# HilaManor/AudioEditingCode

Measured on AMD Instinct MI355X. Metric: edited-clips/sec (200-step inv+edit, 10 s@16 kHz), higher is better.
Workload: dtype f32

## Files before the change

audioeditingcode_amd/csrc/elementwise.hip:

```cpp
#include "aed_common.h"

static inline int grid_for(size_t n, int per_thread = 1) {
    size_t g = (n + 256 * (size_t)per_thread - 1) / (256 * (size_t)per_thread);
    if (g > 4096) g = 4096;
    if (g < 1) g = 1;
    return (int)g;
}

__global__ __launch_bounds__(256) void copy2d_kernel(const float* __restrict__ src, float* __restrict__ dst, int rows,
                                                      int cols, int lds_, int ldd, int vec, const int* state,
                                                      int idx_off, int idx_mul, long idx_stride, const float* coef,
                                                      int c_mul, int c_off, int c_stride, int c_col) {
    const int st = state ? state[0] : 0;
    if (state) src += (size_t)(idx_off + idx_mul * st) * (size_t)idx_stride;
    const float sc = coef ? coef[(size_t)(st * c_mul + c_off) * c_stride + c_col] : 1.0f;
    if (vec) {
        const int q = cols >> 2;
        const size_t total = (size_t)rows * q;
        for (size_t e = (size_t)blockIdx.x * 256 + threadIdx.x; e < total; e += (size_t)gridDim.x * 256) {
            const int r = (int)(e / q);
            const int c = (int)(e - (size_t)r * q) * 4;
            float4 v = *reinterpret_cast<const float4*>(src + (size_t)r * lds_ + c);
            if (coef) { v.x *= sc; v.y *= sc; v.z *= sc; v.w *= sc; }
            *reinterpret_cast<float4*>(dst + (size_t)r * ldd + c) = v;
        }
    } else {
        const size_t total = (size_t)rows * cols;
        for (size_t e = (size_t)blockIdx.x * 256 + threadIdx.x; e < total; e += (size_t)gridDim.x * 256) {
            const int r = (int)(e / cols);
            const int c = (int)(e - (size_t)r * cols);
            const float v = src[(size_t)r * lds_ + c];
            dst[(size_t)r * ldd + c] = coef ? v * sc : v;
        }
    }
}
int launch_copy2d(const aed_op* op, hipStream_t s) {
    const int32_t* i = op->i;
    AED_REQUIRE(op->p[0] && op->p[1], "copy2d: null pointer");
    const int vec = (i[1] % 4 == 0) && (i[2] % 4 == 0) && (i[3] % 4 == 0) && ((uintptr_t)op->p[0] % 16 == 0) &&
                    ((uintptr_t)op->p[1] % 16 == 0) && (i[6] % 4 == 0);
    hipLaunchKernelGGL(copy2d_kernel, dim3(grid_for((size_t)i[0] * i[1] / (vec ? 4 : 1))), dim3(256), 0, s,
                       (const float*)op->p[0], (float*)op->p[1], i[0], i[1], i[2], i[3], vec, (const int*)op->p[2],
                       i[4], i[5], (long)i[6], (const float*)op->p[3], i[7], i[8], i[9], i[10]);
    AED_CHECK_HIP(hipGetLastError());
    return 0;
}

__global__ void time_embed_kernel(float* out, const long long* tt, const int* state, const float* freqs,
                                  const int* row_tidx, int B, int dim, int flip, int ld, int t_imm, int tgroup,
                                  float shift, float max_period, int float_table) {
    const int half = dim / 2;
    const int s = state ? state[0] : 0;
    for (int e = blockIdx.x * blockDim.x + threadIdx.x; e < B * half; e += gridDim.x * blockDim.x) {
        const int b = e / half, i = e - b * half;
        const int ti = s * tgroup + (row_tidx ? row_tidx[b] : 0);
        const float t = !tt ? (float)t_imm : float_table ? reinterpret_cast<const float*>(tt)[ti] : (float)tt[ti];
        const float fr = freqs ? freqs[i] : expf(-logf(max_period) * (float)i / ((float)half - shift));
        const float arg = t * fr;
        const float sv = sinf(arg), cv = cosf(arg);
        float* o = out + (size_t)b * ld;
        if (flip) { o[i] = cv; o[half + i] = sv; }
        else { o[i] = sv; o[half + i] = cv; }
    }
}
int launch_time_embed(const aed_op* op, hipStream_t s) {
    const int32_t* i = op->i;
    AED_REQUIRE(op->p[0] && i[1] % 2 == 0, "time_embed: bad args");
    hipLaunchKernelGGL(time_embed_kernel, dim3(aed_cdiv(i[0] * i[1] / 2, 256)), dim3(256), 0, s, (float*)op->p[0],
                       (const long long*)op->p[1], (const int*)op->p[2], (const float*)op->p[3], (const int*)op->p[4],
                       i[0], i[1], i[2], i[3], i[4], i[5] > 0 ? i[5] : 1, op->f[0],
                       op->f[1] > 0.f ? op->f[1] : 10000.0f, i[6]);
    AED_CHECK_HIP(hipGetLastError());
    return 0;
}

__global__ __launch_bounds__(256) void softmax_rows_kernel(const float* __restrict__ x, float* __restrict__ y, int cols,
                                                            int ldx, int ldy, float scale) {
    __shared__ float red[4];
    const int row = blockIdx.x, tid = threadIdx.x;
    const float* xr = x + (size_t)row * ldx;
    float* yr = y + (size_t)row * ldy;
    float m = -INFINITY;
    for (int c = tid; c < cols; c += 256) m = fmaxf(m, xr[c] * scale);
    for (int o = 32; o > 0; o >>= 1) m = fmaxf(m, __shfl_xor(m, o, 64));
    if ((tid & 63) == 0) red[tid >> 6] = m;
    __syncthreads();
    m = fmaxf(fmaxf(red[0], red[1]), fmaxf(red[2], red[3]));
    __syncthreads();
    float sum = 0.f;
    for (int c = tid; c < cols; c += 256) {
        const float e = expf(xr[c] * scale - m);
        yr[c] = e;
        sum += e;
    }
    for (int o = 32; o > 0; o >>= 1) sum += __shfl_xor(sum, o, 64);
    if ((tid & 63) == 0) red[tid >> 6] = sum;
    __syncthreads();
    sum = (red[0] + red[1]) + (red[2] + red[3]);
    const float inv = 1.0f / sum;
    for (int c = tid; c < cols; c += 256) yr[c] *= inv;
}
int launch_softmax_rows(const aed_op* op, hipStream_t s) {
    const int32_t* i = op->i;
    AED_REQUIRE(op->p[0] && op->p[1], "softmax_rows: null pointer");
    hipLaunchKernelGGL(softmax_rows_kernel, dim3(i[0]), dim3(256), 0, s, (const float*)op->p[0], (float*)op->p[1], i[1],
                       i[2], i[3], op->f[0]);
    AED_CHECK_HIP(hipGetLastError());
    return 0;
}

__global__ __launch_bounds__(256) void transpose_kernel(const float* __restrict__ src, float* __restrict__ dst, int R,
                                                         int C, int lds_, int ldd, long bs_src, long bs_dst) {
    __shared__ float tile[32][33];
    const float* s = src + (size_t)blockIdx.z * bs_src;
    float* d = dst + (size_t)blockIdx.z * bs_dst;
    const int tx = threadIdx.x & 31, ty = threadIdx.x >> 5;
    const int r0 = blockIdx.y * 32, c0 = blockIdx.x * 32;
    for (int j = ty; j < 32; j += 8) {
        const int r = r0 + j, c = c0 + tx;
        tile[j][tx] = (r < R && c < C) ? s[(size_t)r * lds_ + c] : 0.f;
    }
    __syncthreads();
    for (int j = ty; j < 32; j += 8) {
        const int c = c0 + j, r = r0 + tx;
// ... 762 lines not shown
```

audioeditingcode_amd/editing.py:

```python
import math

import torch

from . import _lib as L
from .scheduler import coefficient_table, step_coefficients
from . import tape as tape_mod
from .tape import Tape
from .unet import PackedUNetWeights, UNetEngine

PAD_BIAS = -1.0e30
MASK_BIAS = -10000.0


class Conditioning:

    def __init__(self, ehs0=None, ehs1=None, mask0=None, mask1=None, class_labels=None):
        self.ehs0, self.ehs1, self.mask0, self.mask1, self.class_labels = ehs0, ehs1, mask0, mask1, class_labels

    @property
    def rows(self):
        for t in (self.ehs0, self.ehs1, self.class_labels):
            if t is not None:
                return t.shape[0]
        return 0

    def repeat(self, n):
        f = lambda t: None if t is None else t.repeat_interleave(n, 0) if t.shape[0] == 1 else t
        return Conditioning(f(self.ehs0), f(self.ehs1), f(self.mask0), f(self.mask1), f(self.class_labels))

    def select(self, rows):
        f = lambda t: None if t is None else t[list(rows)]
        return Conditioning(f(self.ehs0), f(self.ehs1), f(self.mask0), f(self.mask1), f(self.class_labels))


def _pad_ctx(parts, L, attr_e, attr_m):
    es, bs = [], []
    dev0 = getattr(parts[0], attr_e).device
    for c in parts:
        e = getattr(c, attr_e).float().to(dev0)
        m = getattr(c, attr_m)
        r, l, d = e.shape
        ep = torch.zeros(r, L, d, dtype=torch.float32, device=e.device)
        ep[:, :l] = e
        b = torch.full((r, L), PAD_BIAS, dtype=torch.float32, device=e.device)
        b[:, :l] = 0.0 if m is None else (1 - m.float().to(e.device)) * MASK_BIAS
        es.append(ep)
        bs.append(b)
    return torch.cat(es, 0), torch.cat(bs, 0)


def variant_plan(tstarts, n_zs, max_variants=None):
    ts = [int(t) for t in tstarts]
    if not ts:
        raise ValueError("edit_variants: the list of variants is empty")
    if max_variants is not None and len(ts) > max_variants:
        raise ValueError(f"edit_variants: {len(ts)} variants in one call, at most {max_variants} "
                         f"(variants.inversion_reverse_variants splits longer lists)")
    for t in ts:
        if not 1 <= t <= n_zs:
            raise ValueError(f"edit_variants: tstart {t} outside [1, {n_zs}] (the number of noise maps zs holds)")
    order = sorted(range(len(ts)), key=lambda v: -ts[v])
    segs, i = [], 0
    while i < len(order):
        j = i
        while j < len(order) and ts[order[j]] == ts[order[i]]:
            j += 1
        segs.append(dict(tstart=ts[order[i]], a=j, join=(i, j)))
        i = j
    for k, sg in enumerate(segs):
        nxt = segs[k + 1]["tstart"] if k + 1 < len(segs) else 0
        sg["start"], sg["steps"] = segs[0]["tstart"] - sg["tstart"], sg["tstart"] - nxt
    return order, segs


def variant_positions(order):
    pos = [0] * len(order)
    for i, v in enumerate(order):
        pos[v] = i
    return pos


def variant_noise(eta_rows):
    if isinstance(eta_rows, float):
        return eta_rows > 0
    if any(e == 0 for e in eta_rows) and any(e != 0 for e in eta_rows):
        raise ValueError("edit_variants: a per-step eta list that is zero at some steps and non-zero at others is not "
                         "supported by the device loop; use inversion_reverse_process per variant")
    return any(e > 0 for e in eta_rows)


# ... 267 lines not shown
                        with lock:
                            g = Tape.graph_capture(body)
                    if plan is not None:
                        plan["graph"] = g
                ev0.record(stream)
                chooser = getattr(self, "lane_chooser", None)
                if chooser is None:
                    for _ in range(steps):
                        Tape.graph_replay(g)
                else:
                    stream = self._replay_in_chunks(g, steps, stream, chooser)
                ev1.record(stream)
                self._last_events = (ev0, ev1)
                if plan is None:
                    stream.synchronize()
                    L.check(L.lib().aed_graph_destroy(g), "aed_graph_destroy")
            else:
                ev0.record(stream)
                for _ in range(steps):
                    body()
                ev1.record(stream)
                self._last_events = (ev0, ev1)
        cur.wait_stream(stream)

    LANE_CHUNK = 5

    def _replay_in_chunks(self, g, steps, stream, chooser):
        pending, cur_s, done = [], stream, 0
        while done < steps:
            if len(pending) >= 2:
                pending.pop(0).synchronize()
            s = chooser() or stream
            if s is not cur_s:
                hand = torch.cuda.Event()
                hand.record(cur_s)
                s.wait_event(hand)
                cur_s = s
            n = min(self.LANE_CHUNK, steps - done)
            with torch.cuda.stream(cur_s):
                for _ in range(n):
                    Tape.graph_replay(g)
            ev = torch.cuda.Event()
            ev.record(cur_s)
            pending.append(ev)
            done += n
        return cur_s

    def last_loop_ms(self):
        ev0, ev1 = self._last_events
        ev1.synchronize()
        return ev0.elapsed_time(ev1)


class EditEngine(LoopPlumbing):
    def __init__(self, unet_cfg, weights, scheduler, device, H, W, kind):
        self.cfg, self.sched, self.device = unet_cfg, scheduler, torch.device(device)
        self.H, self.W, self.C = H, W, unet_cfg["in_channels"]
        self.kind = kind
        self.weights = weights if isinstance(weights, PackedUNetWeights) else PackedUNetWeights(weights, device)
        self.stream = torch.cuda.Stream(device=self.device) if self.device.type == "cuda" else None
        self._unets = {}
        self.state = torch.zeros(4, dtype=torch.int32, device=self.device)
        self.ts_dev = torch.zeros(scheduler.config.num_train_timesteps, dtype=torch.int64, device=self.device)
        self._ts_host = None
        self._plans = {}
        self.max_plans = 8

    def _upload_timesteps(self, ts, n):
        ts = ts.detach().to("cpu", torch.int64).reshape(-1)[:n].clone()
        if self._ts_host is not None and self._ts_host.numel() >= n and torch.equal(self._ts_host[:n], ts):
            return
        self.ts_dev[:n] = ts.to(self.device)
        self._ts_host = ts

    arith = "bf16x6"
    ARITH_MIN_BATCH = 2

    def _arith_for(self, B):
        return self.arith if B >= self.ARITH_MIN_BATCH else "f32"

    SHARE_CFG_ROWS = True
    SHARE_IN_EDIT_LOOP = True

    def unet(self, B, L0=0, L1=0, share=1):
        arith = self._arith_for(B)
        share = int(share) if (self.SHARE_CFG_ROWS and share > 1 and self.kind != "audioldm") else 1
        key = (B, L0, L1) if arith == "f32" else (B, L0, L1, arith)
        if share > 1:
            key = key + (f"share{share}",)
        if key not in self._unets:
            with tape_mod.arith_mode(arith):
                self._unets[key] = UNetEngine(self.cfg, self.weights, self.device, B, self.H, self.W, ctx_len0=L0,
                                              ctx_len1=L1, use_ehs=self.kind != "audioldm",
                                              timesteps_dev=self.ts_dev, state_dev=self.state, share=share)
        return self._unets[key]

    def _set_cond(self, eng, groups, repeat=1):
        tile = (lambda t: t) if repeat == 1 else (lambda t: t.repeat(repeat, *([1] * (t.dim() - 1))))
        if self.kind == "audioldm":
            d0 = groups[0].class_labels.device
            eng.set_conditioning(class_labels=tile(torch.cat([g.class_labels.float().to(d0) for g in groups], 0)))
        elif self.kind == "audioldm2":
            d0 = groups[0].ehs0.device
            e0 = torch.cat([g.ehs0.float().to(d0) for g in groups], 0)
            e1, b1 = _pad_ctx(groups, eng.L1, "ehs1", "mask1")
            eng.set_conditioning(ehs0=tile(e0), ehs1=tile(e1), bias1=tile(b1))
        else:
            e0, b0 = _pad_ctx(groups, eng.L0, "ehs0", "mask0")
            eng.set_conditioning(ehs0=tile(e0), bias0=tile(b0))

    def _coef_table(self, s, ts, eta, kind):
        key = (kind, tuple(int(t) for t in ts), tuple(eta) if isinstance(eta, (list, tuple)) else float(eta),
               int(s.config.num_train_timesteps), int(s.num_inference_steps), str(s.config.prediction_type),
               float(s.alphas_cumprod[0]), float(s.alphas_cumprod[-1]), float(s.final_alpha_cumprod))
        cache = self.__dict__.setdefault("_coef_cache", {})
        tab = cache.pop(key, None)
        if tab is None:
            tab = coefficient_table(s, ts, eta=eta, kind=kind)
            while len(cache) >= 8:
                cache.pop(next(iter(cache)))
        cache[key] = tab
        return tab

    @staticmethod
    def _round_len(n):
        for p2 in (8, 16, 32):
            if n <= p2:
                return p2
        return n

    def _ctx_lens(self, groups):
        if self.kind == "audioldm":
            return 0, 0
        if self.kind == "audioldm2":
            return groups[0].ehs0.shape[1], self._round_len(max(g.ehs1.shape[1] for g in groups))
        return self._round_len(max(g.ehs0.shape[1] for g in groups)), 0

    @torch.inference_mode()
    def to_nhwc(self, x, out=None):
        lead = x.shape[:-3]
        C, H, W = x.shape[-3:]
        src = x.to(self.device, torch.float32).contiguous()
        dst = out if out is not None else torch.empty(*lead, H, W, C, device=self.device, dtype=torch.float32)
        tp = Tape(self.device)
        tp.transpose(src, dst, Bt=max(1, math.prod(lead)), R=C, C=H * W)
        tp.run()
        return dst

    @torch.inference_mode()
    def to_nchw(self, x):
        lead = x.shape[:-3]
        H, W, C = x.shape[-3:]
        src = x.contiguous()
        dst = torch.empty(*lead, C, H, W, device=self.device, dtype=torch.float32)
        tp = Tape(self.device)
        tp.transpose(src, dst, Bt=max(1, math.prod(lead)), R=H * W, C=C)
        tp.run()
        return dst

    @torch.inference_mode()
    def sample_xts(self, x0, noise=None, generator=None):
        s = self.sched
        T = s.num_inference_steps
        x0 = x0.to(self.device, torch.float32).contiguous()
        if noise is None:
            noise = torch.stack([torch.randn(x0.shape, generator=generator, dtype=torch.float32) for _ in range(T)])
        noise = noise.to(self.device, torch.float32).contiguous()
        ts = s.timesteps.cpu()
        abar = s.alphas_cumprod
        t_rows = torch.stack([ts[T - (r + 1)] for r in range(T)])
        sa = (abar[t_rows] ** 0.5).to(self.device)
        sb = ((1 - abar) ** 0.5)[t_rows].to(self.device)
        xts = torch.empty((T + 1, *x0.shape), device=self.device, dtype=torch.float32)
        xts[0] = x0
        L.check(L.lib().aed_sample_xts_from_x0(x0.data_ptr(), noise.data_ptr(), sa.data_ptr(), sb.data_ptr(),
                                                xts[1:].data_ptr(), T, x0.numel(), L.current_stream_ptr()),
                "aed_sample_xts_from_x0")
        return xts

    @staticmethod
    def _etas_in_loop_order(eta, n_rows):
        if not isinstance(eta, (list, tuple)) and not (torch.is_tensor(eta) and eta.dim() > 0):
            return float(eta)
        etas = [float(e) for e in eta]
        if len(etas) < n_rows:
            raise ValueError(f"{len(etas)} eta values for {n_rows} steps")
        return [etas[n_rows - 1 - k] for k in range(n_rows)]

    @torch.inference_mode()
    def invert(self, x0, cond_src, cond_uncond, cfg_src, eta=1.0, numerical_fix=True, noise=None, generator=None,
               xts=None, cfg_tensor=None, mode="sequential", group=8, use_graph=True):
        s = self.sched
        T = s.num_inference_steps
        n = x0.shape[0]
        numel = n * self.C * self.H * self.W
        if xts is None:
            xts = self.sample_xts(x0, noise, generator)
        P = 0 if cond_src is None else cond_src.rows // n
        groups = [cond_uncond.repeat(n)] + ([cond_src] if P else [])
        v_pred = int(s.config.prediction_type == "v_prediction")
        G = 1 if mode == "sequential" else max(1, min(group, T))
        while T % G:
            G -= 1
        rows_per_t = n * (1 + P)
        L0, L1 = self._ctx_lens(groups)
        scalar = float(cfg_src[0]) if (cfg_tensor is None and P) else 1.0
        key = ("invert", n, P, T, G, L0, L1, bool(numerical_fix), v_pred, cfg_tensor is not None, scalar,
               self._arith_for(G * rows_per_t))
        plan = self._get_plan(key)
        if plan is None:
            plan = self._plans[key] = dict(
                state=torch.zeros(4, dtype=torch.int32, device=self.device),
                xts=torch.empty((T + 1, n, self.H, self.W, self.C), device=self.device, dtype=torch.float32),
                zs=torch.zeros((T, n, self.H, self.W, self.C), device=self.device, dtype=torch.float32),
                coef=torch.zeros((T, L.COEF_STRIDE), device=self.device, dtype=torch.float32),
                cfgt=(torch.empty((max(P, 1), n, self.H, self.W, self.C), device=self.device, dtype=torch.float32)
                      if cfg_tensor is not None else None))
            eng = plan["eng"] = self.unet(G * rows_per_t, L0, L1, share=(1 + P) if (n == 1 and G >= 2) else 1)
            pre, post = Tape(self.device), Tape(self.device)
            for g in range(G):
                for blk in range(1 + P):
                    dst = eng.x_in[(g * (1 + P) + blk) * n:(g * (1 + P) + blk + 1) * n]
                    pre.copy2d(plan["xts"], dst, rows=1, cols=numel, ld_src=numel, ld_dst=numel, state=plan["state"],
                               idx_off=T - g, idx_mul=-G, idx_stride=numel, name="x_in<-xts")
            for g in range(G):
                base = g * rows_per_t
                eps_u = eng.eps[base:base + n]
                eps_c = eng.eps[base + n:base + rows_per_t] if P else None
                post.step(L.OP_INVERT_STEP, xts=plan["xts"], zs=plan["zs"], eps_u=eps_u, eps_c=eps_c,
                          cfg=plan["cfgt"], coef=plan["coef"], state=plan["state"], out=None, numel=numel, P=max(P, 1),
                          T=T, v_pred=v_pred, flag=int(numerical_fix), cfg_scalar=scalar, s_mul=G, s_off=g)
            post.advance(plan["state"])
            pre.finalize()
            post.finalize()
            plan["pre"], plan["post"] = pre, post
        eng, pre, post = plan["eng"], plan["pre"], plan["post"]
        xts = self.to_nhwc(xts, out=plan["xts"])
        zs = plan["zs"]
        plan["coef"].copy_(self._coef_table(s, s.timesteps.cpu(), self._etas_in_loop_order(eta, T), "ddpm"))
        self._upload_timesteps(s.timesteps, T)
        if cfg_tensor is not None:
            self.to_nhwc(cfg_tensor.reshape(P, n, self.C, self.H, self.W), out=plan["cfgt"])
        self._set_cond(eng, groups, repeat=G)
        self._patch_time(eng, self.ts_dev, G, rows_per_t, state=plan["state"])
        plan["state"].zero_()

        def body():
            pre.run()
            eng.tape.run()
            post.run()
        self._run_graph(body, T // G, use_graph, plan)
        zs[0].zero_()
        return zs, xts

    def _patch_time(self, eng, ts_dev, G, rows_per_t, offset=0, state=None):
        state = self.state if state is None else state
        op = eng.tape.ops[eng.time_op]
        arr = eng.tape.finalize()
        cache = eng.__dict__.setdefault("_row_tidx_cache", {})
        if rows_per_t not in cache:
            cache[rows_per_t] = (torch.arange(eng.B, dtype=torch.int32) // max(1, rows_per_t)).to(self.device)
        eng._row_tidx = cache[rows_per_t]
        for o in (op, arr[eng.time_op]):
            o.p[1] = ts_dev.data_ptr() + 8 * offset
            o.p[2] = state.data_ptr()
            o.p[4] = eng._row_tidx.data_ptr()
            o.i[5] = G

    @torch.inference_mode()
    def edit(self, xts, zs, tstart, cond_tgt, cond_neg, cfg_tar, eta=1.0, cfg_tensor=None, use_graph=True,
             table_kind="ddpm", n_steps=None):
        s = self.sched
        T = s.num_inference_steps
        n = xts.shape[1]
        numel = n * self.C * self.H * self.W
        Z = int(tstart)
        P = cond_tgt.rows // n
        groups = [cond_neg.repeat(n), cond_tgt]
        ts = s.timesteps.cpu()[T - Z:]
        v_pred = int(s.config.prediction_type == "v_prediction")
        scalar = float(cfg_tar[0]) if cfg_tensor is None else 1.0
        L0, L1 = self._ctx_lens(groups)
        eta_rows = self._etas_in_loop_order(eta, Z)
        any_noise = (eta_rows > 0) if isinstance(eta_rows, float) else any(e > 0 for e in eta_rows)
        has_noise = int(any_noise and zs is not None)
        key = ("edit", n, P, T, Z, L0, L1, v_pred, cfg_tensor is not None, scalar, has_noise, table_kind,
               self._arith_for(n * (1 + P)))
        plan = self._get_plan(key)
        if plan is None:
            plan = self._plans[key] = dict(
                state=torch.zeros(4, dtype=torch.int32, device=self.device),
                cur=torch.empty((n, self.H, self.W, self.C), device=self.device, dtype=torch.float32),
                zs=torch.zeros((Z, n, self.H, self.W, self.C), device=self.device, dtype=torch.float32),
                coef=torch.zeros((Z, L.COEF_STRIDE), device=self.device, dtype=torch.float32),
                cfgt=(torch.empty((P, n, self.H, self.W, self.C), device=self.device, dtype=torch.float32)
                      if cfg_tensor is not None else None))
            eng = plan["eng"] = self.unet(n * (1 + P), L0, L1, share=(1 + P) if (n == 1 and self.SHARE_IN_EDIT_LOOP) else 1)
            pre, post = Tape(self.device), Tape(self.device)
            for blk in range(1 + P):
                pre.copy2d(plan["cur"], eng.x_in[blk * n:(blk + 1) * n], rows=1, cols=numel, ld_src=numel,
                           ld_dst=numel, name="x_in<-x_t")
            post.step(L.OP_REVERSE_STEP, xts=plan["cur"], zs=plan["zs"] if has_noise else None, eps_u=eng.eps[:n],
                      eps_c=eng.eps[n:], cfg=plan["cfgt"], coef=plan["coef"], state=plan["state"], out=plan["cur"],
                      numel=numel, P=P, T=Z if has_noise else 0, v_pred=v_pred, flag=has_noise, cfg_scalar=scalar)
            post.advance(plan["state"])
            pre.finalize()
            post.finalize()
            plan["pre"], plan["post"] = pre, post
        eng, pre, post, cur = plan["eng"], plan["pre"], plan["post"], plan["cur"]
        cur.copy_(xts[Z])
        if has_noise:
            plan["zs"].copy_(zs[:Z])
        plan["coef"].copy_(self._coef_table(s, ts, eta_rows, table_kind))
        self._upload_timesteps(s.timesteps, T)
        if cfg_tensor is not None:
            self.to_nhwc(cfg_tensor.reshape(P, n, self.C, self.H, self.W), out=plan["cfgt"])
        self._set_cond(eng, groups)
        self._patch_time(eng, self.ts_dev, 1, n * (1 + P), offset=T - Z, state=plan["state"])
        plan["state"].zero_()

        def body():
            pre.run()
            eng.tape.run()
            post.run()
        self._run_graph(body, Z if n_steps is None else max(0, min(int(n_steps), Z)), use_graph, plan)
        return cur.clone()

    MAX_VARIANTS = 16

    def _variant_loop(self, tag, order, segs, tgt, neg, cfgs, eta, noise_ok, fill_noise, join_rows, use_graph, src=None,
                      n_tables=0, drift=None, n_steps=None, rowsel=None, seg=None):
        s = self.sched
        T = s.num_inference_steps
        K = len(order)
        Z0 = segs[0]["tstart"]
        eta_rows = self._etas_in_loop_order(eta, Z0)
        has_noise = int(variant_noise(eta_rows) and noise_ok)
        numel = self.C * self.H * self.W
        v_pred = int(s.config.prediction_type == "v_prediction")
        P = 1 if seg is None else seg["P"]
        B = 1 + P
        groups_all = [neg[v] for v in order] + ([tgt[v] for v in order] if seg is None else
                                                [tgt[v].select([j]) for j in range(P) for v in order])
        L0, L1 = self._ctx_lens(groups_all)
        tables = () if src is None else (n_tables,)
        R = None if rowsel is None else len(rowsel["coefs"])
        rkey = () if rowsel is None else (n_tables, R)
        if rowsel is not None:
            tables = (max(n_tables, 1),)
        dkey = () if drift is None else (tuple(drift["vecs"].shape[:2]), drift["s_first"], bool(drift["shift_np"]),
                                          drift["fix_mode"], float(drift["fix_alpha"]))
        key = (tag, K, *(tables if rowsel is None else ()), T, tuple(sg["tstart"] for sg in segs),
               tuple(sg["a"] for sg in segs), L0, L1, v_pred, has_noise,
               tuple(self._arith_for(B * sg["a"]) for sg in segs), *dkey, *rkey, *(() if seg is None else (P,)))
        plan = self._get_plan(key)
        if plan is None:
            plan = self._plans[key] = dict(
                state=torch.zeros(4, dtype=torch.int32, device=self.device),
                cur=torch.empty((K, self.H, self.W, self.C), device=self.device, dtype=torch.float32),
                zs=torch.zeros((*tables, Z0, self.H, self.W, self.C), device=self.device, dtype=torch.float32),
                coef=torch.zeros((*(() if R is None else (R,)), Z0, L.COEF_STRIDE), device=self.device, dtype=torch.float32),
                cfg=torch.zeros(K, device=self.device, dtype=torch.float32),
                src=None if src is None else torch.zeros(K, device=self.device, dtype=torch.int32), segs=[])
            if rowsel is not None:
                plan["rowsel"] = torch.zeros((2, K), device=self.device, dtype=torch.int32)
            if drift is not None:
                S, n_ev = drift["vecs"].shape[:2]
                dev_buf = lambda *shape: torch.zeros(shape, device=self.device, dtype=torch.float32)
                plan.update(vecs=dev_buf(S, n_ev, self.H, self.W, self.C), w=dev_buf(S, K, n_ev),
                            mask=dev_buf(self.H, self.W, self.C) if drift["fix_mode"] else None,
                            par=dev_buf(T + 1, self.H, self.W, self.C) if drift["fix_mode"] == 1 else None)
            if seg is not None:
                lat = (self.H, self.W, self.C)
                plan.update(cfg=torch.zeros((K, P, *lat), device=self.device, dtype=torch.float32),
                            mask=torch.zeros((K, P, *lat), device=self.device, dtype=torch.float32),
                            lag=torch.zeros((K, P), device=self.device, dtype=torch.int32),
                            alpha=torch.zeros(K, device=self.device, dtype=torch.float32),
                            traj=torch.zeros((Z0, *lat), device=self.device, dtype=torch.float32))
            for sg in segs:
                a = sg["a"]
                eng = self.unet(B * a, L0, L1, share=1)
                pre, post = Tape(self.device), Tape(self.device)
# ... 397 lines not shown
```

audioeditingcode_amd/unet.py:

```python
import torch

from . import _lib as L
from .tape import Tape
from .weights import ctx_dims_per_block, _per_block


TWO_SOURCE = True
MERGE_FF2_PROJ = True
FOLD_XATTN = True


def geglu_pack_index(dff):
    q = torch.arange(dff // 32)[:, None]
    j = torch.arange(32)[None, :]
    return torch.cat([32 * q + j, dff + 32 * q + j], 1).reshape(-1)


class PackedUNetWeights:

    def __init__(self, sd, device):
        self.device = torch.device(device)
        self.wd = {}
        self._pack(sd)

    def _dev(self, t):
        return t.contiguous().to(self.device, torch.float32)

    def nbytes(self):
        return sum(v.numel() * 4 for v in self.wd.values())

    def _fold_ln(self, name, w, gamma, beta, bias):
        w64, g64, b64 = w.double(), gamma.double(), beta.double()
        wf = w64 * g64[None, :]
        t = w64 @ b64
        if bias is not None:
            t = t + bias.double()
        self.wd[name + ".weight"] = self._dev(wf.float())
        self.wd[name + ".rowsum"] = self._dev(wf.float().double().sum(1).float())
        self.wd[name + ".t"] = self._dev(t.float())

    def ensure_folded_cross_attention(self, base, H):
        if base + ".xq" in self.wd:
            return
        nrm = base.rsplit(".", 1)[0] + ".norm2"
        wq = self._sd[base + ".to_q.weight"].double()
        wo = self._sd[base + ".to_out.0.weight"].double()
        g, bta = self._sd[nrm + ".weight"].double(), self._sd[nrm + ".bias"].double()
        C = wq.shape[0]
        D = C // H
        wqh = wq.reshape(H, D, C)
        self.wd[base + ".xq"] = self._dev((wqh * g[None, None, :]).permute(0, 2, 1).float())
        self.wd[base + ".xs"] = self._dev(torch.stack([(wqh * g).sum(2), (wqh * bta).sum(2)], 1).float())
        self.wd[base + ".xo"] = self._dev(wo.reshape(C, H, D).permute(1, 0, 2).float())

    def _pack(self, sd):
        wd = self.wd
        self._sd = sd
        temb_w, temb_b, self.temb_off = [], [], {}
        off = 0
        for k, v in sd.items():
            if k.endswith("time_emb_proj.weight"):
                base = k[: -len(".weight")]
                self.temb_off[base] = off
                off += v.shape[0]
                temb_w.append(v)
                temb_b.append(sd[base + ".bias"])
        self.temb_total = off
        wd["temb_all.weight"] = self._dev(torch.cat(temb_w, 0))
        wd["temb_all.bias"] = self._dev(torch.cat(temb_b, 0))
        for k, v in sd.items():
            if "time_emb_proj" in k:
                continue
            if v.dim() == 4:
                v = v.permute(0, 2, 3, 1).reshape(v.shape[0], -1)
            if k.endswith(".to_q.weight"):
                base = k[: -len(".to_q.weight")]
                wq, wk, wv = v, sd[base + ".to_k.weight"], sd[base + ".to_v.weight"]
                blk, which = base.rsplit(".", 1)
                nrm = blk + (".norm1" if which == "attn1" else ".norm2")
                if wk.shape[1] == wq.shape[1]:
                    self._fold_ln(base + ".qkv_ln", torch.cat([wq, wk, wv], 0), sd[nrm + ".weight"], sd[nrm + ".bias"], None)
                self._fold_ln(base + ".q_ln", wq, sd[nrm + ".weight"], sd[nrm + ".bias"], None)
                wd[base + ".kv.weight"] = self._dev(torch.cat([wk, wv], 0))
                continue
            if k.endswith(".ff.net.0.proj.weight"):
                blk = k[: -len(".ff.net.0.proj.weight")]
                dff = v.shape[0] // 2
                if dff % 32:
                    raise NotImplementedError(f"{k}: feed-forward width {dff} is not a multiple of 32")
                perm = geglu_pack_index(dff)
                b1 = sd[blk + ".ff.net.0.proj.bias"]
                self._fold_ln(blk + ".ff1g_ln", v[perm], sd[blk + ".norm3.weight"], sd[blk + ".norm3.bias"], b1[perm])
                continue
            if k.endswith(".ff.net.0.proj.bias") or (".transformer_blocks." in k and k.rsplit(".", 2)[-2].startswith("norm")):
                continue
            if k.endswith(".ff.net.2.weight"):
                blk = k[: -len(".ff.net.2.weight")]
                site = blk[: blk.index(".transformer_blocks")]
                wp = sd[site + ".proj_out.weight"]
                if wp.dim() == 4:
                    wp = wp.reshape(wp.shape[0], -1)
                w2, b2, bp = v.double(), sd[blk + ".ff.net.2.bias"].double(), sd[site + ".proj_out.bias"].double()
                wp = wp.double()
                if w2.shape[1] % 64 == 0:
                    wd[blk + ".ff2_proj.weight"] = self._dev(torch.cat([wp @ w2, wp], 1).float())
                    wd[blk + ".ff2_proj.bias"] = self._dev((wp @ b2 + bp).float())
            if k.endswith(".to_k.weight") or k.endswith(".to_v.weight"):
                continue
            wd[k] = self._dev(v)


class UNetEngine:
    def __init__(self, cfg, weights, device, batch, H, W, ctx_len0=0, ctx_len1=0, use_ehs=True,
                 timesteps_dev=None, state_dev=None, two_source=None, share=1):
        self.cfg = cfg
        self.S = int(share) if (share and share > 1 and batch % int(share) == 0 and
                                cfg.get("class_embed_type") is None) else 1
        self.cB = batch
        self.two_source = TWO_SOURCE if two_source is None else two_source
        self.merge_ff2_proj = MERGE_FF2_PROJ and self.two_source
        self.fold_xattn = FOLD_XATTN
        self.device = torch.device(device)
        self.B, self.H, self.W = batch, H, W
        self.use_ehs = use_ehs
        self.L0, self.L1 = ctx_len0, ctx_len1
        self.timesteps_dev, self.state_dev = timesteps_dev, state_dev
        self.tape = Tape(device)
        self.ctx_tape = Tape(device)
        self._tmp = {}
        self._prefix_idx = []
        _add = self.tape._add

        def counted_add(*a, **k):
            idx = _add(*a, **k)
            if self.cB != self.B:
                self._prefix_idx.append(idx)
            return idx
        self.tape._add = counted_add
        if not isinstance(weights, PackedUNetWeights):
            weights = PackedUNetWeights(weights, device)
        self.weights = weights
        self.wd, self.temb_off, self.temb_total = weights.wd, weights.temb_off, weights.temb_total
        self._build()
        del self.tape._add
        for idx in self._prefix_idx:
            self.tape.meta[idx]["flops"] *= self.S

    def tmp(self, tag, *shape):
        key = (tag, tuple(shape))
        if key not in self._tmp:
            self._tmp[key] = self.tape.alloc(*shape)
        return self._tmp[key]

    def _resnet(self, p, x, Cin, Cout, H, W, dest, groups, eps, x2=None, C1=0):
        tp, wd, B = self.tape, self.wd, self.cB
        h = self.tmp("res_h", B, H, W, Cout)
        off = self.temb_off[p + ".time_emb_proj"]
        a = self.tmp("gn_a", B, H, W, Cin)
        tp.groupnorm(x, wd[p + ".norm1.weight"], wd[p + ".norm1.bias"], a, B=B, HW=H * W, C=Cin, G=groups,
                     eps=eps, act=L.ACT_SILU, x2=x2, C1=C1, name=p + ".norm1")
        tp.conv(a, wd[p + ".conv1.weight"], wd[p + ".conv1.bias"], h, B=B, IH=H, IW=W, Cin=Cin, OH=H, OW=W, N=Cout,
                KH=3, KW=3, pad_h=1, pad_w=1, rowvec=self.temb_all[:, off:off + Cout],
                ld_rv=self.temb_total * (self.B // B),
                name=p + ".conv1")
        a2 = self.tmp("gn_a2", B, H, W, Cout)
        tp.groupnorm(h, wd[p + ".norm2.weight"], wd[p + ".norm2.bias"], a2, B=B, HW=H * W, C=Cout, G=groups,
                     eps=eps, act=L.ACT_SILU, name=p + ".norm2")
        res = x
        if (p + ".conv_shortcut.weight") in wd:
            res = self.tmp("res_sc", B, H, W, Cout)
            tp.conv(x, wd[p + ".conv_shortcut.weight"], wd[p + ".conv_shortcut.bias"], res, B=B, IH=H, IW=W, Cin=Cin,
                    OH=H, OW=W, N=Cout, x2=x2, C1=C1, name=p + ".conv_shortcut")
        else:
            assert x2 is None, "a concatenated input always changes the channel count"
        tp.conv(a2, wd[p + ".conv2.weight"], wd[p + ".conv2.bias"], dest, B=B, IH=H, IW=W, Cin=Cout, OH=H, OW=W,
                N=Cout, KH=3, KW=3, pad_h=1, pad_w=1, res=res, name=p + ".conv2")
        return dest

    def _ln_linear(self, x, pfx, out, M, K, N, name):
        wd = self.wd
        self.tape.linear(x, wd[pfx + ".weight"], wd[pfx + ".t"], out, M=M, K=K, N=N, ln_rowsum=wd[pfx + ".rowsum"],
                         name=name + "+ln")

    def _attn(self, p, x, C, N, heads, out, kv=None, Lk=0, bias=None):
        tp, B = self.tape, self.cB
        M = B * N
        D = C // heads
        if kv is None:
            qkv = self.tmp("t_qkv", M, 3 * C)
            self._ln_linear(x, p + ".qkv_ln", qkv, M, C, 3 * C, p + ".qkv")
            tp.attention(qkv, qkv[:, C:], qkv[:, 2 * C:], out, B=B, H=heads, Nq=N, Nk=N, D=D, ldq=3 * C, ldk=3 * C,
                         ldv=3 * C, ldo=C, bsq=N * 3 * C, bsk=N * 3 * C, bsv=N * 3 * C, bso=N * C,
                         scale=D ** -0.5, name=p + ".sdpa")
        else:
            q = self.tmp("t_q", M, C)
            self._ln_linear(x, p + ".q_ln", q, M, C, C, p + ".q")
            tp.attention(q, kv, kv[:, C:], out, B=B, H=heads, Nq=N, Nk=Lk, D=D, ldq=C, ldk=2 * C, ldv=2 * C, ldo=C,
                         bsq=N * C, bsk=Lk * 2 * C, bsv=Lk * 2 * C, bso=N * C, scale=D ** -0.5, bias=bias,
# ... 12 lines not shown
        b = p + ".transformer_blocks.0"
        o = self.tmp("t_o", M, C)
        self._attn(b + ".attn1", t0, C, N, heads, o)
        t1 = self.tmp("t_1", M, C)
        tp.linear(o, wd[b + ".attn1.to_out.0.weight"], wd[b + ".attn1.to_out.0.bias"], t1, M=M, K=C, N=C, res=t0,
                  name=b + ".attn1.to_out")
        if kind == "self2":
            self._attn(b + ".attn2", t1, C, N, heads, o)
        else:
            which = 0 if kind == "cross0" else 1
            Lk = self.L0 if which == 0 else self.L1
            ctx = self.ehs0 if which == 0 else self.ehs1
            cdim = ctx.shape[-1]
            kv = self.ctx_tape.alloc(B * Lk, 2 * C)
            self.ctx_tape.linear(ctx.view(B * Lk, cdim), wd[b + ".attn2.kv.weight"], None, kv, M=B * Lk, K=cdim,
                                 N=2 * C, name=b + ".attn2.kv")
            bias = self.bias0 if which == 0 else self.bias1
            if self._fold_xattn_ok(C, N, heads, Lk):
                return self._folded_cross_attention(p, b, t1, kv, Lk, bias, C, N, heads, x, dest)
            self._attn(b + ".attn2", t1, C, N, heads, o, kv=kv, Lk=Lk, bias=bias)
        t2 = self.tmp("t_2", M, C)
        tp.linear(o, wd[b + ".attn2.to_out.0.weight"], wd[b + ".attn2.to_out.0.bias"], t2, M=M, K=C, N=C, res=t1,
                  name=b + ".attn2.to_out")
        return self._ff_and_out(p, b, t2, C, M, x, dest)

    def _fold_xattn_ok(self, C, N, heads, Lk):
        return (self.fold_xattn and Lk in (8, 16, 32) and N % 64 == 0 and (heads * Lk) % 32 == 0 and
                self.cB * N <= 4096 and C % 32 == 0)

    def _folded_cross_attention(self, p, b, t1, kv, Lk, kbias, C, N, heads, x, dest):
        tp, ct, wd, B = self.tape, self.ctx_tape, self.wd, self.cB
        base = b + ".attn2"
        self.weights.ensure_folded_cross_attention(base, heads)
        HL, D, M = heads * Lk, C // heads, B * N
        G = ct.alloc(B, HL, C)
        gs = ct.alloc(B, HL, 2)
        VOt = ct.alloc(B, C, HL)
        ct.xattn_fold(kv, wd[base + ".xq"], wd[base + ".xs"], wd[base + ".xo"], G, gs, VOt, B=B, Lk=Lk, H=heads, C=C, D=D,
                      name=base + ".fold")
        P = self.tmp("t_p", M, HL)
        gsf = gs.view(-1)
        tp.conv(t1, G, gsf[1:], P, B=B, IH=N, IW=1, Cin=C, OH=N, OW=1, N=HL, ln_rowsum=gsf, w_bs=HL * C, vec_ld=2,
                vec_bs=HL * 2, sm_group=Lk, sm_scale=D ** -0.5, kbias=kbias, name=base + ".scores+softmax",
                alg_flops=2 * M * C * C + 4 * M * Lk * C)
        t2 = self.tmp("t_2", M, C)
        tp.conv(P, VOt, wd[base + ".to_out.0.bias"], t2, B=B, IH=N, IW=1, Cin=HL, OH=N, OW=1, N=C, res=t1, w_bs=C * HL,
                name=base + ".PV+to_out", alg_flops=2 * M * C * C)
        return self._ff_and_out(p, b, t2, C, M, x, dest)

    def _ff_and_out(self, p, b, t2, C, M, x, dest):
        tp, wd = self.tape, self.wd
        f = self.tmp("t_f", M, 4 * C)
        tp.linear(t2, wd[b + ".ff1g_ln.weight"], wd[b + ".ff1g_ln.t"], f, M=M, K=C, N=8 * C,
                  ln_rowsum=wd[b + ".ff1g_ln.rowsum"], geglu=1, name=b + ".ff1+ln+geglu")
        if self.merge_ff2_proj and (b + ".ff2_proj.weight") in wd:
            tp.linear(f, wd[b + ".ff2_proj.weight"], wd[b + ".ff2_proj.bias"], dest, M=M, K=5 * C, N=C, x2=t2,
                      C1=4 * C, res=x, name=b + ".ff2+proj_out")
            return dest
        t3 = self.tmp("t_3", M, C)
        tp.linear(f, wd[b + ".ff.net.2.weight"], wd[b + ".ff.net.2.bias"], t3, M=M, K=4 * C, N=C, res=t2,
                  name=b + ".ff2")
        tp.linear(t3, wd[p + ".proj_out.weight"], wd[p + ".proj_out.bias"], dest, M=M, K=C, N=C, res=x,
                  name=p + ".proj_out")
        return dest

    def _site(self, prefix, k0, x, C, H, W, heads, dims, groups):
        for j, cdim in enumerate(dims):
            if cdim is None or not self.use_ehs:
                kind = "self2"
            elif self.multi and j > 1:
                kind = "cross1"
            else:
                kind = "cross0"
            if kind != "self2" and self.cB != self.B:
                x = self._expand(x, H, W, C)
            dest = self.tape.alloc(self.cB, H, W, C)
            x = self._transformer(f"{prefix}.attentions.{k0 + j}", x, C, H, W, heads, kind, dest, groups)
        return x

    def _expand(self, x, H, W, C, leave=True):
        S, Bp = self.S, self.B // self.S
        full = self.tape.alloc(self.B, H, W, C)
        n = H * W * C
        for k in range(S):
            self.tape.copy2d(x, full[k:], rows=Bp, cols=n, ld_src=n, ld_dst=S * n, name="cfg_share.expand")
        if leave:
            self.cB = self.B
        return full

    def _build(self):
        cfg, tp, wd, B, H, W = self.cfg, self.tape, self.wd, self.B, self.H, self.W
        boc = cfg["block_out_channels"]
        nb = len(boc)
        lpb = cfg.get("layers_per_block", 2)
        groups = cfg.get("norm_num_groups", 32)
        eps = cfg.get("norm_eps", 1e-5)
        heads_pb = _per_block(cfg.get("num_attention_heads") or cfg.get("attention_head_dim", 8), nb)
        ctx_pb, self.multi = ctx_dims_per_block(cfg)
        cin, cout = cfg["in_channels"], cfg["out_channels"]
        ted = boc[0] * 4
        has_class = cfg.get("class_embed_type") is not None
        concat = bool(cfg.get("class_embeddings_concat"))
        emb_dim = 2 * ted if (has_class and concat) else ted

        self.x_in = tp.alloc(B, H, W, cin, zero=True)
        self.ehs0 = self.ehs1 = self.bias0 = self.bias1 = self.class_labels = None
        if self.use_ehs:
            d0 = [c for blk in ctx_pb for c in blk if c is not None]
            if self.multi:
                dims0 = sorted({blk[1] for blk in ctx_pb if blk[1] is not None})
                dims1 = sorted({blk[2] for blk in ctx_pb if len(blk) > 2 and blk[2] is not None})
                self.ehs0 = tp.alloc(B, self.L0, dims0[0], zero=True)
                self.ehs1 = tp.alloc(B, self.L1, dims1[0], zero=True)
                self.bias1 = tp.alloc(B, self.L1, zero=True)
            else:
                self.ehs0 = tp.alloc(B, self.L0, d0[0], zero=True)
                self.bias0 = tp.alloc(B, self.L0, zero=True)
        if has_class:
            self.class_labels = tp.alloc(B, cfg["projection_class_embeddings_input_dim"], zero=True)

        t_emb = tp.alloc(B, boc[0])
        self.time_op = len(tp.ops)
        tp.time_embed(t_emb, B=B, dim=boc[0], flip=cfg.get("flip_sin_to_cos", True), shift=cfg.get("freq_shift", 0),
                      timesteps=self.timesteps_dev, state=self.state_dev)
        e1 = tp.alloc(B, ted)
        tp.linear(t_emb, wd["time_embedding.linear_1.weight"], wd["time_embedding.linear_1.bias"], e1, M=B,
                  K=boc[0], N=ted, out_act=L.ACT_SILU, name="time_embedding.linear_1")
        self.emb = tp.alloc(B, emb_dim)
        if has_class and not concat:
            cemb = self.ctx_tape.alloc(B, ted)
            self.ctx_tape.linear(self.class_labels, wd["class_embedding.weight"], wd["class_embedding.bias"], cemb,
                                 M=B, K=self.class_labels.shape[1], N=ted, name="class_embedding")
            tp.linear(e1, wd["time_embedding.linear_2.weight"], wd["time_embedding.linear_2.bias"], self.emb, M=B,
                      K=ted, N=ted, res=cemb, name="time_embedding.linear_2")
        else:
            tp.linear(e1, wd["time_embedding.linear_2.weight"], wd["time_embedding.linear_2.bias"], self.emb, M=B,
                      K=ted, N=ted, name="time_embedding.linear_2")
            if has_class:
                self.ctx_tape.linear(self.class_labels, wd["class_embedding.weight"], wd["class_embedding.bias"],
                                     self.emb[:, ted:], M=B, K=self.class_labels.shape[1], N=ted,
                                     name="class_embedding")
        self.temb_all = tp.alloc(B, self.temb_total)
        tp.linear(self.emb, wd["temb_all.weight"], wd["temb_all.bias"], self.temb_all, M=B, K=emb_dim,
                  N=self.temb_total, in_act=L.ACT_SILU, name="time_emb_proj(all resnets)")

        if self.S > 1 and not self.use_ehs:
            self.S = 1
        self.cB = Bc = B // self.S
        h = tp.alloc(Bc, H, W, boc[0])
        tp.conv(self.x_in, wd["conv_in.weight"], wd["conv_in.bias"], h, B=Bc, IH=H, IW=W, Cin=cin, OH=H, OW=W,
                N=boc[0], KH=3, KW=3, pad_h=1, pad_w=1, a_bs=self.S * H * W * cin, name="conv_in")

        def skip_of(t, c_, h_, w_):
            return (t if self.cB == B else self._expand(t, h_, w_, c_, leave=False), c_, h_, w_)
        skips = [skip_of(h, boc[0], H, W)]
        ch, hh, ww = boc[0], H, W
        for i, bt in enumerate(cfg["down_block_types"]):
            co = boc[i]
            for j in range(lpb):
                d = tp.alloc(self.cB, hh, ww, co)
                h = self._resnet(f"down_blocks.{i}.resnets.{j}", h, ch, co, hh, ww, d, groups, eps)
                ch = co
                if "CrossAttn" in bt:
                    h = self._site(f"down_blocks.{i}", j * len(ctx_pb[i]), h, co, hh, ww, heads_pb[i], ctx_pb[i],
                                   groups)
                skips.append(skip_of(h, ch, hh, ww))
            if i < nb - 1:
                oh, ow = (hh + 2 - 3) // 2 + 1, (ww + 2 - 3) // 2 + 1
                d = tp.alloc(self.cB, oh, ow, co)
                p = f"down_blocks.{i}.downsamplers.0.conv"
                tp.conv(h, wd[p + ".weight"], wd[p + ".bias"], d, B=self.cB, IH=hh, IW=ww, Cin=co, OH=oh, OW=ow, N=co,
                        KH=3, KW=3, stride=2, pad_h=1, pad_w=1, name=p)
                h, hh, ww = d, oh, ow
                skips.append(skip_of(h, ch, hh, ww))
        if self.cB != B:
            h = self._expand(h, hh, ww, ch)

        d = tp.alloc(B, hh, ww, ch)
        h = self._resnet("mid_block.resnets.0", h, ch, ch, hh, ww, d, groups, eps)
        h = self._site("mid_block", 0, h, ch, hh, ww, heads_pb[-1], ctx_pb[-1], groups)
        self.h_space = tp.alloc(B, hh, ww, ch)
        self._resnet("mid_block.resnets.1", h, ch, ch, hh, ww, self.h_space, groups, eps)
        h = self.h_space
        self.mid_index = len(tp.ops)
        self.skips = [s[0] for s in skips]

        for i, bt in enumerate(cfg["up_block_types"]):
            lvl = nb - 1 - i
            co = boc[lvl]
            for j in range(lpb + 1):
                sk, sc, sh_, sw_ = skips.pop()
                assert (sh_, sw_) == (hh, ww), "skip / feature-map size mismatch"
                d = tp.alloc(B, hh, ww, co)
                if self.two_source and ch % 64 == 0 and (ch + sc) % 32 == 0 and sc % 4 == 0:
                    h = self._resnet(f"up_blocks.{i}.resnets.{j}", h, ch + sc, co, hh, ww, d, groups, eps, x2=sk, C1=ch)
                else:
                    cat = self.tmp("cat", B, hh, ww, ch + sc)
                    tp.copy2d(h, cat, rows=B * hh * ww, cols=ch, ld_src=h.stride(-2), ld_dst=ch + sc, name="cat.h")
                    tp.copy2d(sk, cat[..., ch:], rows=B * hh * ww, cols=sc, ld_src=sk.stride(-2), ld_dst=ch + sc,
                              name="cat.skip")
                    h = self._resnet(f"up_blocks.{i}.resnets.{j}", cat, ch + sc, co, hh, ww, d, groups, eps)
                ch = co
                if "CrossAttn" in bt:
                    h = self._site(f"up_blocks.{i}", j * len(ctx_pb[lvl]), h, co, hh, ww, heads_pb[lvl], ctx_pb[lvl],
                                   groups)
            if i < nb - 1:
                p = f"up_blocks.{i}.upsamplers.0.conv"
                th, tw = skips[-1][2], skips[-1][3]
                assert th in (2 * hh, 2 * hh - 1) and tw in (2 * ww, 2 * ww - 1)
                d = tp.alloc(B, th, tw, co)
                tp.conv(h, wd[p + ".weight"], wd[p + ".bias"], d, B=B, IH=hh, IW=ww, Cin=co, OH=th, OW=tw,
                        N=co, KH=3, KW=3, pad_h=1, pad_w=1, up=1, name=p)
                h, hh, ww = d, th, tw

        self.eps = tp.alloc(B, hh, ww, cout)
        a = self.tmp("gn_a", B, hh, ww, ch)
        tp.groupnorm(h, wd["conv_norm_out.weight"], wd["conv_norm_out.bias"], a, B=B, HW=hh * ww, C=ch, G=groups,
                     eps=eps, act=L.ACT_SILU, name="conv_norm_out")
        tp.conv(a, wd["conv_out.weight"], wd["conv_out.bias"], self.eps, B=B, IH=hh, IW=ww, Cin=ch, OH=hh, OW=ww,
                N=cout, KH=3, KW=3, pad_h=1, pad_w=1, name="conv_out")
        tp.finalize()
        self.ctx_tape.finalize()

    @torch.inference_mode()
    def set_conditioning(self, ehs0=None, ehs1=None, bias0=None, bias1=None, class_labels=None):
        for dst, src in ((self.ehs0, ehs0), (self.ehs1, ehs1), (self.bias0, bias0), (self.bias1, bias1),
                         (self.class_labels, class_labels)):
            if dst is not None and src is not None:
                dst.copy_(src.to(dst.device, torch.float32).reshape(dst.shape))
        self.ctx_tape.run()

    def set_timestep(self, t):
        self.tape.ops[self.time_op].i[4] = int(t)
        arr = self.tape.finalize()
        arr[self.time_op].i[4] = int(t)

    @torch.inference_mode()
    def forward(self, first_half_only=False, second_half_only=False):
        if second_half_only:
            self.tape.run(self.mid_index, None)
        elif first_half_only:
            self.tape.run(0, self.mid_index)
        else:
            self.tape.run()
        return self.eps
```

Before: 0.9690.

## Precompute timestep embedding table and broadcast-copy it per step

Adds a time-table mode in which the full timestep-embedding MLP (sinusoid, two linears, all-resnet temb projection) runs once for all timesteps into a table. Each UNet step then gathers its row with a state-indexed copy instead of running the chain. It also adds a broadcast path in copy2d (ld_src==0) that reads the source once and writes it to all rows, which the CFG share expand uses. Only one x_in block is copied when rows are shared. This removes several small per-step GEMM launches, at the cost of extra setup logic and a table that must match the step's tile codes.

```diff
diff --git a/audioeditingcode_amd/csrc/elementwise.hip b/audioeditingcode_amd/csrc/elementwise.hip
--- a/audioeditingcode_amd/csrc/elementwise.hip
+++ b/audioeditingcode_amd/csrc/elementwise.hip
@@ -14,7 +14,14 @@
     const int st = state ? state[0] : 0;
     if (state) src += (size_t)(idx_off + idx_mul * st) * (size_t)idx_stride;
     const float sc = coef ? coef[(size_t)(st * c_mul + c_off) * c_stride + c_col] : 1.0f;
-    if (vec) {
+    if (vec && lds_ == 0) {
+        const int q = cols >> 2;
+        for (int e = blockIdx.x * 256 + threadIdx.x; e < q; e += gridDim.x * 256) {
+            float4 v = *reinterpret_cast<const float4*>(src + (size_t)e * 4);
+            if (coef) { v.x *= sc; v.y *= sc; v.z *= sc; v.w *= sc; }
+            for (int r = 0; r < rows; ++r) *reinterpret_cast<float4*>(dst + (size_t)r * ldd + (size_t)e * 4) = v;
+        }
+    } else if (vec) {
         const int q = cols >> 2;
         const size_t total = (size_t)rows * q;
         for (size_t e = (size_t)blockIdx.x * 256 + threadIdx.x; e < total; e += (size_t)gridDim.x * 256) {
@@ -39,7 +46,8 @@
     AED_REQUIRE(op->p[0] && op->p[1], "copy2d: null pointer");
     const int vec = (i[1] % 4 == 0) && (i[2] % 4 == 0) && (i[3] % 4 == 0) && ((uintptr_t)op->p[0] % 16 == 0) &&
                     ((uintptr_t)op->p[1] % 16 == 0) && (i[6] % 4 == 0);
-    hipLaunchKernelGGL(copy2d_kernel, dim3(grid_for((size_t)i[0] * i[1] / (vec ? 4 : 1))), dim3(256), 0, s,
+    const size_t work = (vec && i[2] == 0) ? (size_t)i[1] / 4 : (size_t)i[0] * i[1] / (vec ? 4 : 1);
+    hipLaunchKernelGGL(copy2d_kernel, dim3(grid_for(work)), dim3(256), 0, s,
                        (const float*)op->p[0], (float*)op->p[1], i[0], i[1], i[2], i[3], vec, (const int*)op->p[2],
                        i[4], i[5], (long)i[6], (const float*)op->p[3], i[7], i[8], i[9], i[10]);
     AED_CHECK_HIP(hipGetLastError());
diff --git a/audioeditingcode_amd/editing.py b/audioeditingcode_amd/editing.py
--- a/audioeditingcode_amd/editing.py
+++ b/audioeditingcode_amd/editing.py
@@ -6,6 +6,7 @@
 from .scheduler import coefficient_table, step_coefficients
 from . import tape as tape_mod
 from .tape import Tape
+from . import unet as unet_mod
 from .unet import PackedUNetWeights, UNetEngine
 
 PAD_BIAS = -1.0e30
@@ -439,17 +440,21 @@
     SHARE_CFG_ROWS = True
     SHARE_IN_EDIT_LOOP = True
 
-    def unet(self, B, L0=0, L1=0, share=1):
+    def unet(self, B, L0=0, L1=0, share=1, time_table=False):
         arith = self._arith_for(B)
         share = int(share) if (self.SHARE_CFG_ROWS and share > 1 and self.kind != "audioldm") else 1
+        time_table = bool(time_table and unet_mod.LEAN_STEP and self.cfg.get("class_embed_type") is None)
         key = (B, L0, L1) if arith == "f32" else (B, L0, L1, arith)
         if share > 1:
             key = key + (f"share{share}",)
+        if time_table:
+            key = key + ("time_table",)
         if key not in self._unets:
             with tape_mod.arith_mode(arith):
                 self._unets[key] = UNetEngine(self.cfg, self.weights, self.device, B, self.H, self.W, ctx_len0=L0,
                                               ctx_len1=L1, use_ehs=self.kind != "audioldm",
-                                              timesteps_dev=self.ts_dev, state_dev=self.state, share=share)
+                                              timesteps_dev=self.ts_dev, state_dev=self.state, share=share,
+                                              time_table=time_table)
         return self._unets[key]
 
     def _set_cond(self, eng, groups, repeat=1):
@@ -612,6 +617,10 @@
 
     def _patch_time(self, eng, ts_dev, G, rows_per_t, offset=0, state=None):
         state = self.state if state is None else state
+        if eng.time_table:
+            assert G == 1 and ts_dev is self.ts_dev and ts_dev is eng.timesteps_dev, "time-table engines: one timestep per call"
+            n = int(self._ts_host.numel())
+            return eng.use_time_rows(eng.time_rows(n, version=tuple(self._ts_host.tolist()), timesteps=ts_dev), offset, state)
         op = eng.tape.ops[eng.time_op]
         arr = eng.tape.finalize()
         cache = eng.__dict__.setdefault("_row_tidx_cache", {})
@@ -652,9 +661,10 @@
                 coef=torch.zeros((Z, L.COEF_STRIDE), device=self.device, dtype=torch.float32),
                 cfgt=(torch.empty((P, n, self.H, self.W, self.C), device=self.device, dtype=torch.float32)
                       if cfg_tensor is not None else None))
-            eng = plan["eng"] = self.unet(n * (1 + P), L0, L1, share=(1 + P) if (n == 1 and self.SHARE_IN_EDIT_LOOP) else 1)
+            eng = plan["eng"] = self.unet(n * (1 + P), L0, L1, share=(1 + P) if (n == 1 and self.SHARE_IN_EDIT_LOOP) else 1,
+                                          time_table=True)
             pre, post = Tape(self.device), Tape(self.device)
-            for blk in range(1 + P):
+            for blk in range(1 if (unet_mod.LEAN_STEP and eng.S > 1) else 1 + P):
                 pre.copy2d(plan["cur"], eng.x_in[blk * n:(blk + 1) * n], rows=1, cols=numel, ld_src=numel,
                            ld_dst=numel, name="x_in<-x_t")
             post.step(L.OP_REVERSE_STEP, xts=plan["cur"], zs=plan["zs"] if has_noise else None, eps_u=eng.eps[:n],
diff --git a/audioeditingcode_amd/unet.py b/audioeditingcode_amd/unet.py
--- a/audioeditingcode_amd/unet.py
+++ b/audioeditingcode_amd/unet.py
@@ -8,6 +8,7 @@
 TWO_SOURCE = True
 MERGE_FF2_PROJ = True
 FOLD_XATTN = True
+LEAN_STEP = 1
 
 
 def geglu_pack_index(dff):
@@ -112,8 +113,10 @@
 
 class UNetEngine:
     def __init__(self, cfg, weights, device, batch, H, W, ctx_len0=0, ctx_len1=0, use_ehs=True,
-                 timesteps_dev=None, state_dev=None, two_source=None, share=1):
+                 timesteps_dev=None, state_dev=None, two_source=None, share=1, time_table=False):
         self.cfg = cfg
+        self.time_table = bool(time_table and LEAN_STEP and cfg.get("class_embed_type") is None)
+        self._time_tables = {}
         self.S = int(share) if (share and share > 1 and batch % int(share) == 0 and
                                 cfg.get("class_embed_type") is None) else 1
         self.cB = batch
@@ -292,11 +295,51 @@
         S, Bp = self.S, self.B // self.S
         full = self.tape.alloc(self.B, H, W, C)
         n = H * W * C
-        for k in range(S):
-            self.tape.copy2d(x, full[k:], rows=Bp, cols=n, ld_src=n, ld_dst=S * n, name="cfg_share.expand")
+        if LEAN_STEP and Bp == 1:
+            self.tape.copy2d(x, full, rows=S, cols=n, ld_src=0, ld_dst=n, name="cfg_share.expand")
+        else:
+            for k in range(S):
+                self.tape.copy2d(x, full[k:], rows=Bp, cols=n, ld_src=n, ld_dst=S * n, name="cfg_share.expand")
         if leave:
             self.cB = self.B
         return full
+
+    def _time_chain(self, tp, rows, temb_all, timesteps, state, tiles=(0, 0, 0), row_tidx=None):
+        cfg, wd = self.cfg, self.wd
+        boc = cfg["block_out_channels"]
+        ted = boc[0] * 4
+        has_class = cfg.get("class_embed_type") is not None
+        concat = bool(cfg.get("class_embeddings_concat"))
+        emb_dim = 2 * ted if (has_class and concat) else ted
+        t_emb = tp.alloc(rows, boc[0])
+        time_op = len(tp.ops)
+        tp.time_embed(t_emb, B=rows, dim=boc[0], flip=cfg.get("flip_sin_to_cos", True), shift=cfg.get("freq_shift", 0),
+                      timesteps=timesteps, state=state)
+        if row_tidx is not None:
+            tp.ops[time_op].p[4] = row_tidx.data_ptr()
+            tp.keep.append(row_tidx)
+        e1 = tp.alloc(rows, ted)
+        tp.linear(t_emb, wd["time_embedding.linear_1.weight"], wd["time_embedding.linear_1.bias"], e1, M=rows,
+                  K=boc[0], N=ted, out_act=L.ACT_SILU, tile=tiles[0], name="time_embedding.linear_1")
+        emb = tp.alloc(rows, emb_dim)
+        if has_class and not concat:
+            cemb = self.ctx_tape.alloc(rows, ted)
+            self.ctx_tape.linear(self.class_labels, wd["class_embedding.weight"], wd["class_embedding.bias"], cemb,
+                                 M=rows, K=self.class_labels.shape[1], N=ted, name="class_embedding")
+            tp.linear(e1, wd["time_embedding.linear_2.weight"], wd["time_embedding.linear_2.bias"], emb, M=rows,
+                      K=ted, N=ted, res=cemb, name="time_embedding.linear_2")
+        else:
+            tp.linear(e1, wd["time_embedding.linear_2.weight"], wd["time_embedding.linear_2.bias"], emb, M=rows,
+                      K=ted, N=ted, tile=tiles[1], name="time_embedding.linear_2")
+            if has_class:
+                self.ctx_tape.linear(self.class_labels, wd["class_embedding.weight"], wd["class_embedding.bias"],
+                                     emb[:, ted:], M=rows, K=self.class_labels.shape[1], N=ted,
+                                     name="class_embedding")
+        tp.linear(emb, wd["temb_all.weight"], wd["temb_all.bias"], temb_all, M=rows, K=emb_dim,
+                  N=self.temb_total, in_act=L.ACT_SILU, tile=tiles[2], name="time_emb_proj(all resnets)")
+        if tp is self.tape:
+            self.time_op, self.emb = time_op, emb
+        return time_op
 
     def _build(self):
         cfg, tp, wd, B, H, W = self.cfg, self.tape, self.wd, self.B, self.H, self.W
@@ -308,10 +351,7 @@
         heads_pb = _per_block(cfg.get("num_attention_heads") or cfg.get("attention_head_dim", 8), nb)
         ctx_pb, self.multi = ctx_dims_per_block(cfg)
         cin, cout = cfg["in_channels"], cfg["out_channels"]
-        ted = boc[0] * 4
         has_class = cfg.get("class_embed_type") is not None
-        concat = bool(cfg.get("class_embeddings_concat"))
-        emb_dim = 2 * ted if (has_class and concat) else ted
 
         self.x_in = tp.alloc(B, H, W, cin, zero=True)
         self.ehs0 = self.ehs1 = self.bias0 = self.bias1 = self.class_labels = None
@@ -329,30 +369,18 @@
         if has_class:
             self.class_labels = tp.alloc(B, cfg["projection_class_embeddings_input_dim"], zero=True)
 
-        t_emb = tp.alloc(B, boc[0])
-        self.time_op = len(tp.ops)
-        tp.time_embed(t_emb, B=B, dim=boc[0], flip=cfg.get("flip_sin_to_cos", True), shift=cfg.get("freq_shift", 0),
-                      timesteps=self.timesteps_dev, state=self.state_dev)
-        e1 = tp.alloc(B, ted)
-        tp.linear(t_emb, wd["time_embedding.linear_1.weight"], wd["time_embedding.linear_1.bias"], e1, M=B,
-                  K=boc[0], N=ted, out_act=L.ACT_SILU, name="time_embedding.linear_1")
-        self.emb = tp.alloc(B, emb_dim)
-        if has_class and not concat:
-            cemb = self.ctx_tape.alloc(B, ted)
-            self.ctx_tape.linear(self.class_labels, wd["class_embedding.weight"], wd["class_embedding.bias"], cemb,
-                                 M=B, K=self.class_labels.shape[1], N=ted, name="class_embedding")
-            tp.linear(e1, wd["time_embedding.linear_2.weight"], wd["time_embedding.linear_2.bias"], self.emb, M=B,
-                      K=ted, N=ted, res=cemb, name="time_embedding.linear_2")
-        else:
-            tp.linear(e1, wd["time_embedding.linear_2.weight"], wd["time_embedding.linear_2.bias"], self.emb, M=B,
-                      K=ted, N=ted, name="time_embedding.linear_2")
-            if has_class:
-                self.ctx_tape.linear(self.class_labels, wd["class_embedding.weight"], wd["class_embedding.bias"],
-                                     self.emb[:, ted:], M=B, K=self.class_labels.shape[1], N=ted,
-                                     name="class_embedding")
         self.temb_all = tp.alloc(B, self.temb_total)
-        tp.linear(self.emb, wd["temb_all.weight"], wd["temb_all.bias"], self.temb_all, M=B, K=emb_dim,
-                  N=self.temb_total, in_act=L.ACT_SILU, name="time_emb_proj(all resnets)")
+        if self.time_table:
+            self.time_op = len(tp.ops)
+            tp.copy2d(tp.alloc(1, self.temb_total, zero=True), self.temb_all, rows=B, cols=self.temb_total, ld_src=0,
+                      ld_dst=self.temb_total, state=self.state_dev, idx_off=0, idx_mul=0, idx_stride=self.temb_total,
+                      name="temb_all<-time table")
+            probe = Tape(self.device)
+            self._time_chain(probe, B, probe.alloc(B, self.temb_total), self.timesteps_dev, self.state_dev)
+            self._time_tiles = [int(op.i[29]) for op in probe.ops[1:]]
+            self._time_flags = [int(op.flags) for op in probe.ops[1:]]
+        else:
+            self._time_chain(tp, B, self.temb_all, self.timesteps_dev, self.state_dev)
 
         if self.S > 1 and not self.use_ehs:
             self.S = 1
@@ -440,7 +468,35 @@
                 dst.copy_(src.to(dst.device, torch.float32).reshape(dst.shape))
         self.ctx_tape.run()
 
+    def time_rows(self, n, version=None, timesteps=None, t_imm=0):
+        key = (n, timesteps is None)
+        ent = self._time_tables.get(key)
+        if ent is None:
+            tp = Tape(self.device)
+            table = tp.alloc(n, self.temb_total)
+            ridx = torch.arange(n, dtype=torch.int32).to(self.device)
+            top = self._time_chain(tp, n, table, timesteps, None, tiles=self._time_tiles, row_tidx=ridx)
+            got = [(int(op.i[29]), int(op.flags)) for op in tp.ops[top + 1:]]
+            assert got == list(zip(self._time_tiles, self._time_flags)), \
+                f"time table: tile codes / flags {got} differ from the step's {self._time_tiles} / {self._time_flags}"
+            ent = self._time_tables[key] = dict(tape=tp, table=table, top=top, version=object())
+        if timesteps is None:
+            ent["tape"].ops[ent["top"]].i[4] = int(t_imm)
+            ent["tape"].finalize()[ent["top"]].i[4] = int(t_imm)
+        if ent["version"] != version or timesteps is None:
+            ent["tape"].run()
+            ent["version"] = version
+        return ent["table"]
+
+    def use_time_rows(self, table, offset=0, state=None, step=1):
+        for o in (self.tape.ops[self.time_op], self.tape.finalize()[self.time_op]):
+            o.p[0] = table.data_ptr()
+            o.p[2] = None if state is None else state.data_ptr()
+            o.i[4], o.i[5] = int(offset), int(step)
+
     def set_timestep(self, t):
+        if self.time_table:
+            return self.use_time_rows(self.time_rows(1, t_imm=t))
         self.tape.ops[self.time_op].i[4] = int(t)
         arr = self.tape.finalize()
         arr[self.time_op].i[4] = int(t)
```

New measurement: 0.9660, median of 5. Within noise of the previous version (-0.3%).
